# hkbharath/MARL-MASS

Hardware: AMD Instinct MI355X
Metric: agent-steps/sec (whole node), MASS CBF shield on, 65536 envs x 8 CAVs (higher is better)
Workload: dtype f64

## Files before the change

marl-mass_amd/csrc/mm_kernels.hip:

```cpp
#include <hip/hip_runtime.h>
#include <math.h>
#include <stdio.h>
#include <string.h>

#include <type_traits>

#include "mm_device.h"
#include "mm_div.h"
#include "mm_handle.h"
#define MM_COUNTS_FN __host__ __device__ inline
#include "../../include/mm_counts.h"
#include "../../include/mm_policy_wide.h"
#include "../../include/mm_env_params.h"

using namespace mm;

struct DevCfg {
  int env_kind, shield, nsub, T, action_masking, auto_reset, obs_f64, N, E, debug_flags, n_hdv;
  double dt, collision_reward, high_speed_reward, headway_cost, headway_time, merging_lane_cost;
  double rs_lo, rs_hi, eta, tau;
  double inv_dt, rs_span, rs_ispan, rs_span2, rs_ispan2;
  int agent_reward;
  int steer_vel;
  int *err;
// ... 1307 lines not shown
  } else {
    return c;
  }
}
template <int G, int SHIELD, bool MIXED>
#ifndef MM_GENERAL_NONE_WAVES
#define MM_GENERAL_NONE_WAVES 3
#endif
constexpr int step_min_waves(bool ipm = false) { return SHIELD == MM_SHIELD_NONE ? (G >= MM_NONE_WIDE_G ? 2 : (MIXED ? MM_GENERAL_NONE_WAVES : MM_NONE_WAVES)) : (ipm ? (G >= 6 ? MM_IPM_WIDE_WAVES : (MIXED ? MM_IPM_WAVES : MM_IPM_CAV_WAVES)) : MM_MIN_WAVES); }
template <int G, int KIND, int SHIELD, bool MIXED, bool IPM = false, bool TRACE = false, bool SPLIT = false, bool PENV = false>
#ifndef MM_STEP_BLOCK
#define MM_STEP_BLOCK 64
#endif
__global__ __launch_bounds__(MM_STEP_BLOCK, (SPLIT ? MM_SPLIT_WAVES : step_min_waves<G, SHIELD, MIXED>(IPM))) void step_kernel(DevCfg c, DevState st, const int32_t *__restrict__ actions,
                                                   MMStepOut out, double *metrics, SweepBuf sb, int kb, PoseBuf pb) {
  constexpr bool IDM = kIdm<KIND>;
  constexpr bool LC = (KIND == MM_ENV_V1) || IDM;
  constexpr bool SHIELDED = LC && (SHIELD != MM_SHIELD_NONE);
  static_assert(!IDM || (MIXED && SHIELD == MM_SHIELD_NONE && !IPM && !SPLIT), "hdv-v1: general unshielded kernels only");
  constexpr bool MASS = (SHIELD == MM_SHIELD_MASS);
  static_assert(!IPM || SHIELDED, "the IPM mode lives in shielded kernels");
  static_assert(!SPLIT || IPM, "the split form exists for the interior-point kernels");
  static_assert(!PENV || (SHIELDED && KIND == MM_ENV_V1 && !TRACE && !SPLIT), "per-env parameters: fused shielded v1 kernels without the trace");
#ifdef MM_SERIAL_ALL
  constexpr bool kSerialOnly = true || IPM;
#else
#ifdef MM_SERIAL_MASS
  constexpr bool kSerialOnly = MIXED || MASS || IPM;
#else
  constexpr bool kSerialOnly = MIXED;
#endif
#endif
  constexpr bool kSine = SHIELDED && !SPLIT && !MIXED && !IPM && !kSerialOnly && kPow2<G> && G <= 8;
  constexpr bool kScan = kScanSelects && !MIXED && !TRACE;
#ifndef MM_CARRY_POSE
#define MM_CARRY_POSE 1
#endif
  constexpr bool kCarry = kSine && MM_CARRY_POSE != 0;
#ifndef MM_PRIMARY_PRIOR
#define MM_PRIMARY_PRIOR 1
#endif
  constexpr bool kPrimary = kSine && !TRACE && kVetoPrior && MM_PRIMARY_PRIOR != 0;
#ifndef MM_SINE_CARRY
#define MM_SINE_CARRY 0
#endif
  constexpr bool kSineCarry = kPrimary && MM_SINE_CARRY != 0;
#ifndef MM_ACT_FRAME
#define MM_ACT_FRAME 1
#endif
  constexpr bool kActSel = kPrimary && MM_ACT_FRAME != 0;
  constexpr bool kEarly = kSine && MM_EARLY_LOADS != 0;
  constexpr bool kHBits = kSine && !TRACE && kPoseHBits;
  constexpr bool kWideObs = kSine && !TRACE && kObsWide;
  double car_sn = __builtin_nan("");
  (void)car_sn;
  static_assert(kPow2<G> || MM_STEP_BLOCK == 64, "rotation layouts: one wave per workgroup");
  const long long gtid = (long long)blockIdx.x * blockDim.x + threadIdx.x;
  constexpr int kTail = kPow2<G> ? 64 : (64 / G) * G;
  const bool tail = lane_id() >= kTail;
  const int gb = kPow2<G> ? (lane_id() & ~(G - 1)) : (tail ? kTail - G : lane_id() - lane_id() % G);
  const int a = kPow2<G> ? (int)(gtid % G) : lane_id() - gb;
  const long long e = kPow2<G> ? gtid / G : (tail ? (long long)st.E : (gtid >> 6) * (64 / G) + lane_id() / G);
  const bool valid = e < st.E && a < st.N;
  const long long i = e * st.N + a;
  const long long A = st.A;
  const double dt = c.dt;

#ifdef MM_STAMPS
  const unsigned long long _rec_t0 = __builtin_amdgcn_s_memtime(), _rec_rt0 = __builtin_amdgcn_s_memrealtime();
  unsigned long long _t_last = __builtin_amdgcn_s_memtime(), _t_acc = 0;
#endif
  Veh v;
  const bool sv = MIXED && KIND == MM_ENV_V1 && c.steer_vel != 0;
  int steps = 0, time = 0, n_merge = 0, episode = 0;
  int car_code = 0;
  long long car_kx = 0, car_ky = 0, car_kh = 0;
  double car_s = 0.0, car_c = 1.0;
  int act_raw = 1;
  (void)act_raw;
  if constexpr (kEarly) {
    if (valid) act_raw = actions[i];
    if (e < st.E) { n_merge = st.I[MM_E_N_MERGE * st.E + e]; episode = st.I[MM_E_EPISODE * st.E + e]; }
  }
  if constexpr (kCarry) {
    if (valid) {
      car_kx = __double_as_longlong(pb.F[PB_KX * A + i]); car_ky = __double_as_longlong(pb.F[PB_KY * A + i]);
      car_kh = __double_as_longlong(pb.F[PB_KH * A + i]);
      car_s = pb.F[PB_SIN * A + i]; car_c = pb.F[PB_COS * A + i]; car_code = pb.code[i];
    }
  }
  load_veh(st, i, valid, v, sv);
  if (e < st.E) {
    steps = st.I[MM_E_STEPS * st.E + e]; time = st.I[MM_E_TIME * st.E + e];
  }
  if (!MIXED && v.kind == 2) v.kind = 1;
  if (IDM && v.present) v.kind = 2;
  const bool hdv = MIXED && v.kind == 2;
  const bool ctrl = IDM ? v.present : (v.present && !hdv);
  const bool ctrl_x = IDM ? false : ctrl;
  int action;
  if constexpr (kEarly) action = ctrl ? act_raw : 1;
  else action = (!IDM && valid && ctrl) ? actions[i] : 1;
  if ((unsigned)action > 4u) {
    if (!SPLIT || kb == 0) atomicOr(c.err, MM_LATCH_BAD_ACTION);
    action = 1;
  }
  const unsigned present_bits = group_ballot<G>(v.present, gb);
  const unsigned ctrl_bits = group_ballot<G>(ctrl, gb);
  const int n_veh = __popc(present_bits), n_ctrl = __popc(ctrl_bits);
  if (!SPLIT || kb == 0) steps += 1;

  double cpsi = 1.0, spsi = 0.0;
  double st_t = __builtin_nan("");
  int pk_self = v.lane;
  bool carried = false;
  if constexpr (kCarry) {
    const bool hit = car_kx == __double_as_longlong(v.x) && car_ky == __double_as_longlong(v.y) && car_kh == __double_as_longlong(v.h) &&
                     (car_code >> 8) == ((kPoseWritten >> 8) | (MASS ? 1 : 0)) && (car_code & 7) == v.lane;
    carried = !__any(v.present && !hit);
    if (carried && v.present) { spsi = car_s; cpsi = car_c; pk_self = (car_code & 0xFF) | (kHBits ? pose_hbits(v.h) : 0); }
  }
  if (!carried) {
    if (v.present) mmm_sincos(v.h, &spsi, &cpsi);
    if (SHIELDED && v.present) pk_self = pose_code(v.lane, next_lane(v.lane, v.x, v.y), MASS ? corner_flags<kSine>(v.x, v.y, spsi, cpsi, v.lane) : 0);
    if constexpr (kHBits) { if (v.present) pk_self |= pose_hbits(v.h); }
  }

  enum { C_B = 0, C_H1X = 8, C_H1VX, C_H2X, C_H2VX, C_SSTEER, C_SACC, C_TSPEED, C_A = 15, C_GU0 = 23, C_GU1 = 24, C_PRE = 25, C_MSGW = 29 };
  constexpr bool kMailbox = G <= 8 || !kPow2<G>;
  constexpr bool kPackMsg = !kPow2<G>;
  constexpr int kColdB = kMailbox ? (kPackMsg ? 29 : 30) : 25;
  constexpr bool kRoomy = false;
  constexpr int C_CPSI = kColdB + G - 1, C_GVX = C_CPSI + 1;
  constexpr int kColdN = !SHIELDED ? 15 : (kSerialOnly ? 23 : kColdB + G - 1 + (kRoomy ? 2 : 0));
  static_assert(kColdN * MM_STEP_BLOCK * 8 >= (MM_STEP_BLOCK / 64) * 64 * 30 * 4, "the obs staging must fit in the cold slots");
  __shared__ alignas(kWideObs ? 16 : 8) double s_cold[kColdN][MM_STEP_BLOCK];
  const int tid = threadIdx.x;
  auto cold_i = [&](int slot, int col) -> int & { return ((int *)&s_cold[slot][col])[0]; };
  if (LC) {
    s_cold[C_H1X][tid] = v.h1x; s_cold[C_H1VX][tid] = v.h1vx; s_cold[C_H2X][tid] = v.h2x; s_cold[C_H2VX][tid] = v.h2vx;
    s_cold[C_SSTEER][tid] = v.safe_steer; s_cold[C_SACC][tid] = v.safe_acc;
  }
  s_cold[C_TSPEED][tid] = v.tspeed;
  if constexpr (kEarly) {
    static_assert(kMailbox && !kPackMsg, "the high words of the pose-code and rank-word slots must be free");
    ((int *)&s_cold[C_PRE + 3][tid])[1] = n_merge; ((int *)&s_cold[C_MSGW][tid])[1] = episode;
  }
  if constexpr (kRoomy) { s_cold[C_CPSI][tid] = cpsi; s_cold[C_GVX][tid] = v.gvx; }
  auto CPSI = [&]() -> double { if constexpr (kRoomy) return s_cold[C_CPSI][tid]; else return cpsi; };
  auto GVX = [&]() -> double { if constexpr (kRoomy) return s_cold[C_GVX][tid]; else return v.gvx; };
  bool env_active = IDM ? n_veh > 0 : n_ctrl > 0;
  if constexpr (SPLIT) {
    if (kb > 0) env_active = e < st.E && sb.envf[e] != 0;
  }
  STAMP(0);
  const int k_lo = SPLIT ? (kb > 0 ? kb - 1 : 0) : 0, k_hi = SPLIT ? (kb < c.nsub ? kb : c.nsub - 1) : c.nsub - 1;
  for (int k = k_lo; k <= k_hi; k++) {
    const bool head = !SPLIT || k == kb, tail = !SPLIT || k != kb;
    const bool live = env_active && v.present;
    QpTrace qt = {0, __builtin_nan(""), __builtin_nan(""), __builtin_nan(""), __builtin_nan(""),
                  __builtin_nan(""), __builtin_nan(""), __builtin_nan("")};
    int rank = 0;
    if ((SHIELDED || MIXED) && head) {
      for_partners<G>([&](auto mc) {
        constexpr int m = decltype(mc)::value;
        double px = px_d<m, G>(v.x, a);
        bool pp = px_i<m, G>((int)live, a) != 0;
        if constexpr (kScan) rank += (pp & ((px > v.x) | ((px == v.x) & (pidx<m, G>(a) < a)))) ? 1 : 0;
        else rank += (pp && (px > v.x || (px == v.x && pidx<m, G>(a) < a))) ? 1 : 0;
      });
    }
    if (head) v.tspeed = s_cold[C_TSPEED][tid];
    if constexpr (kActSel) {
      Veh w = v;
      if (time % c.nsub == 0) hl_act<KIND>(w, action);
      controlled_act<false, kSine>(w, -1, sv, st_t);
      v.hl = live ? w.hl : v.hl; v.sidx = live ? w.sidx : v.sidx; v.tspeed = live ? w.tspeed : v.tspeed;
      v.tlane = live ? w.tlane : v.tlane; v.act_acc = live ? w.act_acc : v.act_acc;
    } else {
      if (live && !hdv && head) {
        if (time % c.nsub == 0) hl_act<KIND>(v, action);
      }
    }
    const int tl_pre = v.tlane;
    if constexpr (!kActSel) {
      if (live && !hdv && head) controlled_act<!MIXED && !kPrimary, kSine>(v, -1, sv, st_t);
    }
    if (head) s_cold[C_TSPEED][tid] = v.tspeed;
    if constexpr (MIXED) { STAMP(1); }
    if constexpr (MIXED) {
      if (head && __any(hdv && live)) {
        const bool acting = hdv && live && !v.crashed;
        double koff = 0.0, koff_obst = 0.0;
        if (__any(acting && v.lane == MM_LANE_KB0)) {
          koff = kSineAmp * mmm_sin(kSinePuls * (v.x - lane_sx(MM_LANE_KB0)) + kSinePhase);
          koff_obst = kSineAmp * mmm_sin(kSinePuls * (kObstX - lane_sx(MM_LANE_KB0)) + kSinePhase);
        }
        Body self = {true, false, v.x, v.y, v.h, v.v, v.tspeed, v.lane, spsi, cpsi, koff};
        const double s_me = v.x - lane_sx(v.lane);
        NbSel n0 = {0, 0, -1, -1}, n1 = {0, 0, -1, -1};
        const LaneFrame lf0 = lane_frame(v.lane);
        if (acting && lane_after_end(v.tlane, v.x)) v.tlane = next_lane(v.tlane, v.x, v.y);
        const int my_tl = v.tlane;
        const bool lc_branch = v.lane != my_tl;
        const bool same_road = lane_road(v.lane) == lane_road(my_tl);
        const bool timer_due = !lc_branch && (1.0 < v.gvx);
        const int side = v.lane == MM_LANE_BC0 ? MM_LANE_BC1 : (v.lane == MM_LANE_BC1 ? MM_LANE_BC0 : -1);
        const bool try_mobil = acting && timer_due && side >= 0 && lane_reachable(side < 0 ? 0 : side, v.x, v.y);
        const int sl = side < 0 ? 0 : side;
        const double s_side = v.x - lane_sx(sl);
        const LaneFrame lf1 = lane_frame(sl);
        unsigned abort_mask = 0;
        for_partners<G>([&](auto mc) {
          constexpr int m = decltype(mc)::value;
          const int p = pidx<m, G>(a);
          const bool bp = px_i<m, G>((int)live, a) != 0;
          const double bx = px_d<m, G>(v.x, a), by = px_d<m, G>(v.y, a), bk = px_d<m, G>(koff, a);
          if (acting) {
            neighbour_update(lf0, s_me, bp, bx, by, bk, p, n0);
            if (try_mobil) neighbour_update(lf1, s_side, bp, bx, by, bk, p, n1);
          }
          if (__any(acting && lc_branch && same_road)) {
            Body b = {bp, false, bx, by, 0.0, px_d<m, G>(v.v, a), 0.0, px_i<m, G>(v.lane, a), px_d<m, G>(spsi, a), px_d<m, G>(cpsi, a), bk};
// ... 42 lines not shown
            const int p_tl = ((pk & 15) < rank) ? ((pk >> 8) & 7) : ((pk >> 4) & 7);
            hit = hit || (((abort_mask >> p) & 1u) && p_tl == my_tl);
          });
          const int nxt = (acting && lc_branch) ? ((same_road && hit) ? v.lane : my_tl) : tl_post;
          const bool changed = nxt != tl_post;
          tl_post = nxt;
          if (!__any(changed)) break;
        }
        if constexpr (MIXED) { STAMP(5); }
        if (acting) {
          v.tlane = tl_post;
          v.act_acc = clipd(acc_f0, -6.0, 6.0);
        }
      }
      if (head && live && (!hdv || !v.crashed)) steer_lane(v, sv && !hdv, st_t);
      if (head && hdv && live) v.gvx += dt;
    }
    bool first_B = false;
    if constexpr (kPrimary) {
      static_assert(!MIXED && !SPLIT, "kPrimary: no HDVs, no steer_vel, every launch a whole step");
      first_B = (c.debug_flags & 1) == 0 && live && v.hist_len >= 2 && (v.tlane != v.lane || v.crashed) && !(v.flags & MM_FLAG_IS_LC_SAFE);
      if (live) {
        const int tl_1 = v.tlane + (first_B ? v.lane - v.tlane : 0);
        const double steer = steering_control<kSine, kSineCarry>(v.x, v.y, v.h, v.v, tl_1, st_t, car_sn);
        v.act_steer = clipd(steer, -kPi / 3, kPi / 3);
        const double steer_1 = v.act_steer, st_t_1 = st_t;
        clip_actions<kSine>(v, LC, st_t);
        if (first_B) { v.act_steer = steer_1; st_t = st_t_1; }
      }
    } else {
      if (live && head) clip_actions<kSine>(v, LC && !hdv, st_t);
    }
    STAMP(1);
    Cand cA;
    memset(&cA, 0, sizeof cA);
    const bool shield_on = SHIELDED && live && !hdv && v.hist_len >= 2;
    if constexpr (kSineCarry) car_sn = __builtin_nan("");
    if (live && head) cA = predict<KIND, SHIELDED, MASS, MIXED, kSine, kHBits>(v, v.act_steer, st_t, spsi, cpsi, dt, sv && !hdv, kSineCarry ? &car_sn : nullptr);
    auto park = [&](auto base_c, const Cand &cc, double steer) {
      constexpr int base = decltype(base_c)::value;
      if constexpr (SHIELDED) {
        s_cold[base + 0][tid] = cc.x; s_cold[base + 1][tid] = cc.y; s_cold[base + 2][tid] = cc.h;
        cold_i(base + 3, tid) = cc.pk; s_cold[base + 4][tid] = cc.cpsi; s_cold[base + 5][tid] = steer;
        s_cold[base + 6][tid] = cc.gvx; s_cold[base + 7][tid] = cc.spsi;
      }
    };
    auto park_at = [&](int base, const Cand &cc, double steer) {
      s_cold[base + 0][tid] = cc.x; s_cold[base + 1][tid] = cc.y; s_cold[base + 2][tid] = cc.h;
      cold_i(base + 3, tid) = cc.pk; s_cold[base + 4][tid] = cc.cpsi; s_cold[base + 5][tid] = steer;
      s_cold[base + 6][tid] = cc.gvx; s_cold[base + 7][tid] = cc.spsi;
    };
    if constexpr (kPrimary) park_at(first_B ? (int)C_B : (int)C_A, cA, v.act_steer);
    else if (head) park(std::integral_constant<int, C_A>{}, cA, v.act_steer);
    STAMP(2);
    const bool needB = SHIELDED && shield_on && (v.tlane != v.lane || v.crashed || sv);
    bool haveB = first_B, haveA = !first_B;
    (void)haveA;
    auto make_other = [&]() {
      if constexpr (kPrimary) {
        const bool mk_A = !haveA;
        if (mk_A || (needB && !haveB)) {
          double t_o;
          const int tl_o = v.lane + (mk_A ? v.tlane - v.lane : 0);
          double steer_o = steering_control<kSine>(v.x, v.y, v.h, v.v, tl_o, t_o);
          if (mk_A) {
            steer_o = clipd(steer_o, -kPi / 3, kPi / 3);
            if (v.crashed) { steer_o = 0; t_o = 0; }
          }
          park_at(mk_A ? (int)C_A : (int)C_B, predict<KIND, true, MASS, MIXED, kSine, kHBits>(v, steer_o, t_o, spsi, cpsi, dt, false), steer_o);
          haveA = true; haveB = haveB || !mk_A;
        }
      }
    };
    auto make_B = [&]() {
      if constexpr (SHIELDED) {
        if (needB && !haveB) {
          double tB;
          double steerB = steering_control<kSine>(v.x, v.y, v.h, v.v, v.lane, tB);
          if (sv) steerB = steer_vel_command(steerB, v.sang);
          park(std::integral_constant<int, C_B>{}, predict<KIND, true, MASS, MIXED, kSine, kHBits>(v, steerB, tB, spsi, CPSI(), dt, sv), steerB);
          haveB = true;
        }
      }
    };
    auto chosen = [&](bool useB) {
      if constexpr (!SHIELDED) {
        return cA;
      } else {
        const int base = useB ? C_B : C_A;
        Cand cc;
        cc.x = s_cold[base + 0][tid]; cc.y = s_cold[base + 1][tid]; cc.h = s_cold[base + 2][tid];
        cc.gvx = s_cold[base + 6][tid]; cc.cpsi = s_cold[base + 4][tid]; cc.spsi = s_cold[base + 7][tid];
        const int pk = cold_i(base + 3, tid);
        cc.pk = pk; cc.lane = pk & 7;
        return cc;
      }
    };
    if constexpr (SPLIT) {
      if (!head && live && valid) {
        v.act_acc = sw_f(sb, SW_ACCN, a, e);
        if (MIXED && hdv) {
          v.act_steer = sw_f(sb, SW_ASTEER, a, e);
          if (sw_i(sb, SW_RES, a, e) & 16) s_cold[C_H1X][tid] = sw_f(sb, SW_ACC, a, e);
        }
        s_cold[C_A + 0][tid] = sw_f(sb, SW_AX, a, e); s_cold[C_A + 1][tid] = sw_f(sb, SW_AY, a, e); s_cold[C_A + 2][tid] = sw_f(sb, SW_AH, a, e);
        cold_i(C_A + 3, tid) = sw_i(sb, SW_APK, a, e); s_cold[C_A + 4][tid] = sw_f(sb, SW_ACPSI, a, e); s_cold[C_A + 5][tid] = sw_f(sb, SW_ASTEER, a, e);
// ... 14 lines not shown
#endif
    if constexpr (kPrimary) {
      use_B = first_B;
#ifdef MM_STAMPS
      st_prior = first_B;
#endif
      CAND_COUNT(MM_CS_FIRST_B, first_B);
    } else if constexpr (SHIELDED && !SPLIT && !kSerialOnly && kVetoPrior) {
      CAND_COUNT(MM_CS_UPFRONT, (c.debug_flags & 1) == 0 && shield_on && needB && !(v.flags & MM_FLAG_IS_LC_SAFE));
      if ((c.debug_flags & 1) == 0 && shield_on && needB && !(v.flags & MM_FLAG_IS_LC_SAFE)) { make_B(); use_B = true; }
#ifdef MM_STAMPS
      st_prior = use_B;
#endif
    }
    STAMP(MM_CS_UPFRONT_CYCLES);
    if constexpr (SPLIT) {
      if (head) {
        make_B();
        if constexpr (!kSerialOnly && kVetoPrior) use_B = (c.debug_flags & 1) == 0 && shield_on && needB && !(v.flags & MM_FLAG_IS_LC_SAFE);
        const int n_live = __popc(group_ballot<G>(live, gb));
        if (valid) {
          sw_i(sb, SW_META, a, e) = (live ? 1 : 0) | (shield_on ? 2 : 0) | (needB ? 4 : 0) | (hdv ? 8 : 0) | (use_B ? 16 : 0) | (v.flags & 255) << 8 | (v.hl & 255) << 16;
          if (live) {
            sw_i(sb, SW_WPK, a, e) = pk_self;
            sw_f(sb, SW_CPSI, a, e) = cpsi; sw_f(sb, SW_ACCN, a, e) = v.act_acc;
            sw_f(sb, SW_AX, a, e) = cA.x; sw_f(sb, SW_AY, a, e) = cA.y; sw_f(sb, SW_AH, a, e) = cA.h; sw_i(sb, SW_APK, a, e) = cA.pk;
            sw_f(sb, SW_ACPSI, a, e) = cA.cpsi; sw_f(sb, SW_AGVX, a, e) = cA.gvx; sw_f(sb, SW_ASTEER, a, e) = v.act_steer; sw_f(sb, SW_ASPSI, a, e) = cA.spsi;
            if (needB) {
              sw_f(sb, SW_BX, a, e) = s_cold[C_B + 0][tid]; sw_f(sb, SW_BY, a, e) = s_cold[C_B + 1][tid]; sw_f(sb, SW_BH, a, e) = s_cold[C_B + 2][tid];
              sw_i(sb, SW_BPK, a, e) = cold_i(C_B + 3, tid); sw_f(sb, SW_BCPSI, a, e) = s_cold[C_B + 4][tid]; sw_f(sb, SW_BSTEER, a, e) = s_cold[C_B + 5][tid];
              sw_f(sb, SW_BGVX, a, e) = s_cold[C_B + 6][tid]; sw_f(sb, SW_BSPSI, a, e) = s_cold[C_B + 7][tid];
            }
            sb.order[(long long)rank * sb.Ep + e] = (uint8_t)a;
          }
          if (a >= n_live) sb.order[(long long)a * sb.Ep + e] = 0xFF;
          if (a == 0) sb.envf[e] = env_active ? 1 : 0;
        }
      } else if (shield_on && valid) {
        const int res = sw_i(sb, SW_RES, a, e);
        new_acc = sw_f(sb, SW_ACC, a, e); veto = (res & 2) != 0; use_B = (res & 4) != 0; new_flags = (res >> 8) & 255;
      }
    }

    if constexpr (SHIELDED) {
     if (__any(shield_on) && (!SPLIT || head)) {
      bool serial = !SPLIT && (kSerialOnly || (c.debug_flags & 1) != 0);
      ShieldOut so;
      memset(&so, 0, sizeof so);
      if constexpr (!kSerialOnly) {
       if (!serial) {
        static_assert(!MIXED || kSerialOnly, "the parallel form is CAV-only (the twin branch needs the literal sweep)");
        bool irregular = false;
        constexpr bool count5 = G > 4;
        if constexpr (kMailbox) { s_cold[C_PRE + 0][tid] = v.x; s_cold[C_PRE + 1][tid] = v.y; s_cold[C_PRE + 2][tid] = v.h; cold_i(C_PRE + 3, tid) = pk_self; }
        double qc_h0 = 0.0, qc_h3 = 0.0, qc_d = 0.0;
        int qc_meta = 0;
        (void)qc_h0; (void)qc_h3; (void)qc_d; (void)qc_meta;
        for (int pass = 0; pass <= st.N; pass++) {
#ifdef MM_STAMPS
#ifdef MM_COUNT_ROUNDS
          if ((threadIdx.x & 63) == 13) _t_acc += (pass == 0 ? 1ull << 32 : 0ull);
#else
          if ((threadIdx.x & 63) == 13) _t_acc += 1 + (pass == 0 ? 1ull << 32 : 0ull);
#endif
#endif
          const double mine_gvx = s_cold[(use_B ? C_B : C_A) + 6][tid];
          const double h1vx_mine = s_cold[C_H1VX][tid];
          s_cold[C_GU0][tid] = slot_gu<MASS>(s_cold[C_H2VX][tid], MASS ? s_cold[C_SACC][tid] : kCbfAccLo, GVX(), dt);
          s_cold[C_GU1][tid] = slot_gu<MASS>(h1vx_mine, kCbfAccLo, mine_gvx, dt);
          if constexpr (kMailbox) {
            const int my_word = (live ? rank : 99) | (use_B ? 256 : 0);
            if constexpr (kPackMsg) ((int *)&s_cold[C_PRE + 3][tid])[1] = my_word;
            else cold_i(C_MSGW, tid) = my_word;
            __builtin_amdgcn_fence(__ATOMIC_RELEASE, "wavefront");
            __builtin_amdgcn_wave_barrier();
            __builtin_amdgcn_fence(__ATOMIC_ACQUIRE, "wavefront");
          }
          Cand mine;
          if constexpr (!kMailbox) mine = chosen(use_B);
          double k_ol = INFINITY, k_oa = INFINITY, k_oar = INFINITY;
          int j_ol = -1, j_oa = -1, j_oar = -1;
          for_partners<G>([&](auto mc) {
            constexpr int m = decltype(mc)::value;
            const int p = pidx<m, G>(a);
            int p_rank, opk;
            double ox, oy, oh;
            bool i_first;
            if constexpr (kMailbox) {
              const int pl = plane<m, G>(tid, a);
              int pw;
              if constexpr (kPackMsg) pw = ((const int *)&s_cold[C_PRE + 3][pl])[1];
              else pw = cold_i(C_MSGW, pl);
              p_rank = pw & 255;
              i_first = live && rank < p_rank;
              const int pb = (!i_first && p_rank < 99) ? ((pw & 256) ? (int)C_B : (int)C_A) : (int)C_PRE;
              ox = s_cold[pb + 0][pl]; oy = s_cold[pb + 1][pl];
              if constexpr (kHBits) oh = 0.0;
              else oh = s_cold[pb + 2][pl];
              opk = cold_i(pb + 3, pl) | (p_rank < 99 ? 256 : 0);
            } else {
              p_rank = dppx_i<m>(live ? rank : 99);
              i_first = live && rank < p_rank;
              const double sx_ = i_first ? mine.x : v.x, sy_ = i_first ? mine.y : v.y, sh_ = i_first ? mine.h : v.h;
              const int spk = i_first ? mine.pk : pk_self;
              ox = dppx_d<m>(sx_); oy = dppx_d<m>(sy_); oh = dppx_d<m>(sh_);
              opk = dppx_i<m>(spk | (int)live << 8);
            }
            const bool o_first = !i_first && p_rank < 99;
            const Rel r = relate<kHBits && kMailbox>(v.x, v.y, pk_self, ((opk >> 8) & 1) != 0, ox, oy, oh, opk);
            if constexpr (count5) s_cold[kColdB + m - 1][tid] = r.key;
            const bool b_ol = (r.cls == 1) & ((r.key < k_ol) | ((r.key == k_ol) & (p < (j_ol & 15))));
            const bool b_oa = (r.cls == 2) & ((r.key < k_oa) | ((r.key == k_oa) & (p < (j_oa & 15))));
            const bool b_oar = (r.cls == 3) & ((r.key < k_oar) | ((r.key == k_oar) & (p < (j_oar & 15))));
            const int pf = p | (o_first ? 16 : 0) | (r.cflag ? 32 : 0);
            k_ol = b_ol ? r.key : k_ol; j_ol = b_ol ? pf : j_ol;
            k_oa = b_oa ? r.key : k_oa; j_oa = b_oa ? pf : j_oa;
            k_oar = b_oar ? r.key : k_oar; j_oar = b_oar ? pf : j_oar;
          });
          const bool ol_first = j_ol >= 0 && (j_ol & 16), oa_first = j_oa >= 0 && (j_oa & 16), oar_stepped = j_oar >= 0 && (j_oar & 16);
          const bool cadj = j_oa >= 0 && (j_oa & 32);
          j_ol = j_ol < 0 ? -1 : (j_ol & 15); j_oa = j_oa < 0 ? -1 : (j_oa & 15); j_oar = j_oar < 0 ? -1 : (j_oar & 15);
          STAMP(3);
          Neigh nb;
          memset(&nb, 0, sizeof nb);
          nb.has_ol = j_ol >= 0; nb.has_oa = j_oa >= 0; nb.has_oar = j_oar >= 0;
          if constexpr (count5) {
            int pos_ol = 0, pos_oa = 0, pos_oar = 0;
#pragma unroll
            for (int m = 1; m < G; m++) {
              const int p = pidx_rt<G>(a, m);
              const double km = s_cold[kColdB + m - 1][tid];
              pos_ol += (km < k_ol || (km == k_ol && p < j_ol)) ? 1 : 0;
              pos_oa += (km < k_oa || (km == k_oa && p < j_oa)) ? 1 : 0;
              pos_oar += (km < k_oar || (km == k_oar && p < j_oar)) ? 1 : 0;
            }
            nb.has_ol = nb.has_ol && pos_ol < 5;
            nb.has_oa = nb.has_oa && pos_oa < 5;
            nb.has_oar = nb.has_oar && pos_oar < 5;
          }
          nb.constrain_adj = MASS && nb.has_oa && cadj;
          if constexpr (SPLIT) {
            if (valid && shield_on)
              sw_i(sb, SW_CLS, a, e) = (j_ol & 15) | (j_oa & 15) << 4 | (j_oar & 15) << 8 | (nb.has_ol ? 1 << 12 : 0) | (nb.has_oa ? 1 << 13 : 0) |
                                       (nb.has_oar ? 1 << 14 : 0) | (nb.constrain_adj ? 1 << 15 : 0);
            break;
          }
          __builtin_amdgcn_fence(__ATOMIC_RELEASE, "wavefront");
          __builtin_amdgcn_wave_barrier();
          __builtin_amdgcn_fence(__ATOMIC_ACQUIRE, "wavefront");
          const int t_ol = tid - a + (j_ol < 0 ? a : j_ol), t_oa = tid - a + (j_oa < 0 ? a : j_oa);
          nb.ol_x = s_cold[ol_first ? C_H1X : C_H2X][t_ol]; nb.ol_gu = s_cold[ol_first ? C_GU1 : C_GU0][t_ol];
          nb.oa_x = s_cold[oa_first ? C_H1X : C_H2X][t_oa]; nb.oa_gu = s_cold[oa_first ? C_GU1 : C_GU0][t_oa];
          const int src_ol = gb + (j_ol < 0 ? 0 : j_ol), src_oa = gb + (j_oa < 0 ? 0 : j_oa), src_oar = gb + (j_oar < 0 ? 0 : j_oar);
          const double cpsi_now = CPSI();
          nb.oar_x = shfl_d(v.x, src_oar); nb.oar_vx = shfl_d(v.v * cpsi_now, src_oar);
          bool ol_dyn = MASS && nb.has_ol && ol_first, oa_dyn = MASS && nb.has_oa && oa_first;
          {
            unsigned rep = obstacle_override<MASS>(nb, v.x, v.y);
            if (rep & 1u) ol_dyn = false;
            if (rep & 2u) oa_dyn = false;
          }
          irregular = irregular || (shield_on && nb.has_oar && oar_stepped);
// ... 83 lines not shown
#endif
            for (int round = 0; round <= st.N; round++) {
#if defined(MM_STAMPS) && defined(MM_COUNT_ROUNDS)
              if ((threadIdx.x & 63) == 13) _t_acc += 1;
#endif
              CAND_COUNT(MM_CS_ROUNDS, shield_on);
              const double gu_cur = slot_gu<true>(h1vx_mine, acc_cur, mine_gvx, dt);
              const double da = shfl_d(gu_cur, src_ol), db = shfl_d(gu_cur, src_oa);
              if (ol_dyn) nb.ol_gu = da;
              if (oa_dyn) nb.oa_gu = db;
              rr = shield_rows<true>(c, ss, nb);
              d_cur = qp_exact(ss, rr);
              double acc_next = v.act_acc;
              if (shield_on) {
                if (slow_lc) acc_next = shield_post<true>(env_cfg<PENV>(c, e, st.E), v, ss, rr, d_cur, true, false).acc;
                else acc_next = div_c((ss.u0 + d_cur) - ss.evx, dt, c.inv_dt);
              }
              const bool changed = __double_as_longlong(acc_next) != __double_as_longlong(acc_cur);
              acc_cur = acc_next;
              if (!__any(changed)) break;
            }
            so = shield_post<true>(env_cfg<PENV>(c, e, st.E), v, ss, rr, d_cur, true, false);
            STAMP(MM_CS_ROUND_CYCLES);
          } else {
          for (int round = 0; round <= st.N; round++) {
            if (MASS) {
              const double gu_cur = slot_gu<true>(h1vx_mine, acc_cur, mine_gvx, dt);
              const double da = shfl_d(gu_cur, src_ol), db = shfl_d(gu_cur, src_oa);
              if (ol_dyn) nb.ol_gu = da;
              if (oa_dyn) nb.oa_gu = db;
            }
            so = shield_dyn<MASS, true, false>(env_cfg<PENV>(c, e, st.E), v, ss, nb, shield_on);
            const double acc_next = shield_on ? so.acc : v.act_acc;
            const bool changed = __double_as_longlong(acc_next) != __double_as_longlong(acc_cur);
            acc_cur = acc_next;
            if (!MASS || !__any(changed)) break;
          }
          }
          }
          if (TRACE && shield_on) trace_status(out.trace + (long long)k * MM_T_COUNT * A + i, A, so);
          STAMP(4);
          const bool want_B = shield_on && so.veto && needB;
          CAND_COUNT(MM_CS_LAZY_B, want_B && !haveB);
          if constexpr (kPrimary) {
            CAND_COUNT(MM_CS_LAZY_A, !want_B && !haveA);
            if (want_B ? !haveB : !haveA) make_other();
          } else {
            if (want_B) make_B();
          }
          STAMP(5);
          const bool flip = want_B != use_B;
          use_B = want_B;
          if (!__any(flip)) break;
        }
        serial = __any(irregular);
        if (!serial && shield_on) {
          new_acc = so.acc; veto = so.veto; new_flags = so.flags; qt = so.qt;
          if (IPM && so.bounds) atomicOr(c.err, MM_LATCH_QP_BOUNDS);
        }
       }
      }
      if (!SPLIT && serial) {
        CAND_COUNT(MM_CS_FALLBACK, !haveA || (needB && !haveB));
        if constexpr (kPrimary) make_other();
        else make_B();
        use_B = false; veto = false; new_acc = v.act_acc; new_flags = v.flags;
        if constexpr (kRoomy) { v.gvx = GVX(); cpsi = CPSI(); }
        double wx = v.x, wy = v.y, wh = v.h, wg = hdv ? 1.0 : v.gvx, wacc = hdv ? kCbfAccLo : s_cold[C_SACC][tid], wvx = v.v * cpsi;
        double whx = s_cold[C_H2X][tid], whvx = s_cold[C_H2VX][tid];
        int wpk = pk_self;
        if (MIXED && hdv && live) {
        }
        double wgu = slot_gu<MASS>(whvx, MASS ? wacc : kCbfAccLo, wg, dt);
        bool w_stepped = false;
        double twin_shift = 0;
        int srank = 0;
        for_partners<G>([&](auto mc) {
          constexpr int m = decltype(mc)::value;
          srank += (px_i<m, G>(shield_on ? rank : 99, a) < rank) ? 1 : 0;
        });
        for (int j = 0; j < st.N; j++) {
          const unsigned sel = group_ballot<G>(shield_on && srank == j, gb);
          if (!__any(sel != 0)) break;
          const bool has = sel != 0;
          const int ai = has ? (__ffs((int)sel) - 1) : 0;
          const int src = gb + ai;
          if constexpr (MIXED) {
            const int r_ego = shfl_i(rank, src);
            if (live && hdv && has && rank < r_ego && !w_stepped) {
              const Cand ca = chosen(false);
              wx = ca.x; wy = ca.y; wh = ca.h; wpk = ca.pk;
              whx = s_cold[C_H1X][tid]; whvx = s_cold[C_H1VX][tid]; w_stepped = true; twin_shift = 0;
              wgu = slot_gu<MASS>(whvx, MASS ? wacc : kCbfAccLo, wg, dt);
            }
          }
          const double ex = shfl_d(v.x, src), ey = shfl_d(v.y, src);
          const int epk = shfl_i(pk_self, src);
          const double e_vx = shfl_d(v.v * cpsi, src);
          const Rel rl = relate(ex, ey, epk, live && has && a != ai, wx, wy, wh, wpk, hdv);
          int pos = 0;
          for_partners<G>([&](auto mc) {
            constexpr int m = decltype(mc)::value;
            double kp = px_d<m, G>(rl.key, a);
            pos += (kp < rl.key || (kp == rl.key && pidx<m, G>(a) < a)) ? 1 : 0;
          });
          const bool in5 = rl.key < INFINITY && pos < 5;
// ... 72 lines not shown
    CAND_COUNT(MM_CS_PRIOR_HELD, st_prior && use_B);
    CAND_COUNT(MM_CS_PRIOR_LIFTED, st_prior && !use_B);
    if (SPLIT && SHIELDED && out.trace && live && tail && !shield_on) {
      out.trace[(long long)k * MM_T_COUNT * A + i + MM_T_QP_ROWS * A] = 0;
    }
    if (!SPLIT && SHIELDED && TRACE && live) {
      double *t = out.trace + (long long)k * MM_T_COUNT * A + i;
      t[MM_T_QP_ROWS * A] = qt.rows; t[MM_T_QP_A * A] = qt.a;
      t[MM_T_QP_H0 * A] = qt.h0; t[MM_T_QP_H1 * A] = qt.h1; t[MM_T_QP_H2 * A] = qt.h2;
      t[MM_T_QP_H3 * A] = qt.h3; t[MM_T_QP_D * A] = qt.d; t[MM_T_LC_MARGIN * A] = qt.margin;
    }
    if (tail) {
    if constexpr (kSineCarry) {
      if (!(live && use_B == first_B)) car_sn = __builtin_nan("");
    }
    if (live) {
      const Cand cc = chosen(use_B);
      const double acc = (SHIELDED && shield_on) ? new_acc : v.act_acc;
      double nv = v.v + acc * dt;
      nv = nv > 0 ? nv : 0;
      if (SHIELDED && shield_on) {
        if (veto) v.tlane = v.lane;
        v.flags = new_flags;
      }
      v.x = cc.x; v.y = cc.y; v.h = cc.h; v.v = nv; v.lane = cc.lane;
      if (LC) {
        if (!hdv) {
          double steer_nom = v.act_steer;
          if constexpr (SHIELDED) steer_nom = s_cold[C_A + 5][tid];
          s_cold[C_SSTEER][tid] = (SHIELDED && shield_on && veto && haveB) ? s_cold[C_B + 5][tid] : steer_nom;
          s_cold[C_SACC][tid] = acc; v.gvx = cc.gvx;
          if constexpr (kRoomy) s_cold[C_GVX][tid] = cc.gvx;
          if (sv) v.sang += s_cold[C_SSTEER][tid] * dt;
        }
        s_cold[C_H2X][tid] = s_cold[C_H1X][tid]; s_cold[C_H2VX][tid] = s_cold[C_H1VX][tid];
        s_cold[C_H1X][tid] = v.x; s_cold[C_H1VX][tid] = v.v * cc.cpsi;
        if (v.hist_len < 2) v.hist_len++;
      }
      if constexpr (kRoomy) s_cold[C_CPSI][tid] = cc.cpsi;
      else cpsi = cc.cpsi;
      spsi = cc.spsi;
      if (SHIELDED) pk_self = cc.pk;
    }

    STAMP(7);
    unsigned need = 0;
#ifdef MM_STAMPS
    bool near_any = false;
    CAND_COUNT(MM_CS_PRECHECK, live);
#endif
    for_partners<G>([&](auto mc) {
      constexpr int m = decltype(mc)::value;
      double px = px_d<m, G>(v.x, a), py = px_d<m, G>(v.y, a), ph = px_d<m, G>(v.h, a);
      bool pp = px_i<m, G>((int)live, a) != 0;
      double dx = px - v.x, dy = py - v.y;
      const bool near = live & pp & !((dx * dx + dy * dy) > kU5);
      CAND_COUNT(MM_CS_NEAR, near);
#ifdef MM_STAMPS
      near_any |= near;
#endif
      need |= (near & boxes_may_touch(dx, dy, v.h, ph, 0.9 * kVehLength / 2, 0.9 * kVehWidth / 2)) ? 1u << pidx<m, G>(a) : 0u;
    });
    CAND_COUNT(MM_CS_NEAR_ANY, near_any);
    {
      double dx = kObstX - v.x, dy = kObstY - v.y;
      const bool near = live & !((dx * dx + dy * dy) > kU5);
      need |= (near & boxes_may_touch(dx, dy, v.h, 0.0, 0.9 * 2.0 / 2, 0.9 * 2.0 / 2)) ? 1u << G : 0u;
    }
    unsigned hits = 0;
    bool obst_hit = false;
    if (__any(need != 0)) {
      for (int p = 0; p <= G; p++) {
        const bool t = ((need >> p) & 1u) != 0;
        if (!__any(t)) continue;
        const bool is_obst = p == G;
        const int src = gb + (is_obst ? 0 : p);
        double px = shfl_d(v.x, src), py = shfl_d(v.y, src), ph = shfl_d(v.h, src);
        if (is_obst) { px = kObstX; py = kObstY; ph = 0.0; }
        const double ol = is_obst ? 2.0 : kVehLength, ow = is_obst ? 2.0 : kVehWidth;
        if (t && rects_intersect(v.x, v.y, v.h, px, py, ol, ow, ph)) {
          if (is_obst) obst_hit = true;
          else hits |= 1u << p;
        }
      }
    }
    if (__any(hits != 0 || obst_hit)) {
      unsigned cb = group_ballot<G>(v.crashed != 0, gb);
      const unsigned ob = group_ballot<G>(obst_hit, gb);
      for (int ii = 0; ii < st.N; ii++) {
        const unsigned row = (unsigned)shfl_i((int)hits, gb + ii);
        for (int jj = 0; jj < st.N; jj++) {
          const double si = shfl_d(v.v, gb + ii), sj = shfl_d(v.v, gb + jj);
          const bool fire = !((cb >> ii) & 1u) && ii != jj && ((row >> jj) & 1u);
          if (fire) {
            const double s = fabs(si) <= fabs(sj) ? si : sj;
            if (a == ii || a == jj) { v.v = s; v.crashed = 1; }
            cb |= (1u << ii) | (1u << jj);
          }
        }
        if (!((cb >> ii) & 1u) && ((ob >> ii) & 1u)) {
          if (a == ii) { v.v = fabs(v.v) <= 0 ? v.v : 0.0; v.crashed = 1; }
          cb |= 1u << ii;
        }
      }
    }
    STAMP(8);
    if (env_active) time += 1;
// ... 88 lines not shown
  double local = 0;
  if (ctrl) {
    const bool xrew = LC && c.agent_reward != 0, is_mrew = c.agent_reward == 2;
    const bool half = xrew && is_mrew && (v.flags & MM_FLAG_IS_COLLABORATING);
    double scaled = 0 + (half ? div_c((v.v - c.rs_lo) * (1 - 0), c.rs_span2, c.rs_ispan2)
                              : div_c((v.v - c.rs_lo) * (1 - 0), c.rs_span, c.rs_ispan));
    double merging = 0;
    if (v.lane == MM_LANE_BC1 && (!(xrew && is_mrew) || (v.flags & MM_FLAG_IS_LC_SAFE))) {
      double t = v.x - 420;
      merging = -mmm_exp(MM_DIVC(-(t * t), 1000.0));
    }
    double hc = v.v > 0 ? mmm_log(hd / (env_cfg<PENV>(c, e, st.E).headway_time * v.v)) : 0;
    if (xrew) hc = -1 * hc;
    local = c.collision_reward * (-1 * v.crashed) + (c.high_speed_reward * clipd(scaled, 0, 1)) +
            c.merging_lane_cost * merging + c.headway_cost * (hc < 0 ? hc : 0);
  }
  double regional = 0;
  {
    const bool on_main = v.lane == MM_LANE_AB0 || v.lane == MM_LANE_BC0 || v.lane == MM_LANE_CD0;
    const int i_fl = on_main ? of_i : sf_i, i_rl = on_main ? or_i : sr_i;
    const int i_fr = on_main ? sf_i : of_i, i_rr = on_main ? sr_i : or_i;
    const double r_fl = shfl_d(local, gb + (i_fl < 0 ? 0 : i_fl)), r_fr = shfl_d(local, gb + (i_fr < 0 ? 0 : i_fr));
    const double r_rl = shfl_d(local, gb + (i_rl < 0 ? 0 : i_rl)), r_rr = shfl_d(local, gb + (i_rr < 0 ? 0 : i_rr));
    auto is_mdp = [&](int j) { return j >= 0 && !((hdv_bits >> j) & 1u); };
    double sum = 0;
    int cnt = 0;
    if (is_mdp(i_fl)) { sum += r_fl; cnt++; }
    if (is_mdp(i_fr)) { sum += r_fr; cnt++; }
    sum += local; cnt++;
    if (is_mdp(i_rl)) { sum += r_rl; cnt++; }
    if (is_mdp(i_rr)) { sum += r_rr; cnt++; }
    regional = sum / cnt;
  }
  double rsum = 0, ssum = 0, tsum = 0;
#pragma unroll
  for (int q = 0; q < G; q++) {
    const double lr = shfl_d(local, gb + q), sp = shfl_d(v.v, gb + q);
    const bool in = q < st.N, cq = in & (((ctrl_bits >> q) & 1u) != 0), pq = in & (((present_bits >> q) & 1u) != 0);
    const double r1 = rsum + lr, s1 = ssum + sp, t1 = tsum + sp;
    rsum = cq ? r1 : rsum; ssum = cq ? s1 : ssum;
    tsum = pq ? t1 : tsum;
  }
  const double reward = env_ok ? rsum / n_ctrl : 0, avg_speed = env_ok ? ssum / n_ctrl : 0;
  const double traffic_speed = env_ok ? tsum / n_veh : 0;
  double th = INFINITY;
  if (ctrl) {
    double h2d = hd;
    if (fabs(kObstY - v.y) <= 2 && kObstX > v.x) { double dd = kObstX - v.x; if (dd < h2d) h2d = dd; }
    h2d = h2d - kVehLength;
    double vx = v.v * cpsi;
    th = h2d / (vx > 1 ? vx : 1);
  }
  const double min_headway = group_min_d<G>(th, a);
  if constexpr (kEarly) { n_merge = ((const int *)&s_cold[C_PRE + 3][tid])[1]; episode = ((const int *)&s_cold[C_MSGW][tid])[1]; }
  else if (e < st.E) { n_merge = st.I[MM_E_N_MERGE * st.E + e]; episode = st.I[MM_E_EPISODE * st.E + e]; }
  double merge_pct = __builtin_nan("");
  if (done) {
    const int n_rem = __popc(group_ballot<G>(
        ctrl && (v.lane == MM_LANE_BC1 || v.lane == MM_LANE_KB0 || v.lane == MM_LANE_JK0), gb));
    merge_pct = n_merge > 0 ? (double)(n_merge - n_rem) / n_merge * 100 : 100.0;
  }
  if (valid) {
    if (out.agents_rewards) out.agents_rewards[i] = ctrl ? local : 0;
    if (out.regional_rewards) out.regional_rewards[i] = ctrl ? regional : 0;
    if (out.agents_dones) out.agents_dones[i] = ctrl ? (uint8_t)(v.crashed || steps >= c.T || v.x < 0) : 1;
    if (out.crashed) out.crashed[i] = v.present ? (uint8_t)v.crashed : 0;
    if (out.agents_info) {
      out.agents_info[i * 3 + 0] = v.present ? v.x : 0;
      out.agents_info[i * 3 + 1] = v.present ? v.y : 0;
      out.agents_info[i * 3 + 2] = v.present ? v.v : 0;
    }
  }
  if (e < st.E && a == 0 && env_ok) {
    if (out.reward) out.reward[e] = reward;
    if (out.done) out.done[e] = (uint8_t)done;
    if (out.average_speed) out.average_speed[e] = avg_speed;
    if (out.traffic_speed) out.traffic_speed[e] = traffic_speed;
    if (out.min_headway) out.min_headway[e] = min_headway;
    if (out.merge_percent) out.merge_percent[e] = merge_pct;
  }
  STAMP(10);
  if (metrics) {
    static_assert(MM_STEP_BLOCK % 64 == 0, "whole waves per workgroup");
    const bool lead = e < st.E && a == 0 && env_ok;
    const double mv[8] = {lead ? reward : 0.0, (lead && done && crashed_bits) ? 1.0 : 0.0, lead ? avg_speed : 0.0,
                          lead ? traffic_speed : 0.0, lead ? 1.0 : 0.0, (lead && done) ? merge_pct : 0.0,
                          (lead && done) ? 1.0 : 0.0, lead ? min_headway : INFINITY};
    if (a == 0) {
#pragma unroll
      for (int k = 0; k < 8; k++) s_cold[C_B + k][tid] = mv[k];
    }
    __builtin_amdgcn_fence(__ATOMIC_RELEASE, "wavefront");
    __builtin_amdgcn_wave_barrier();
    __builtin_amdgcn_fence(__ATOMIC_ACQUIRE, "wavefront");
    const int ln = lane_id();
    if (ln < 8) {
      const int slot = C_B + ln, base = tid - ln;
      double acc = ln == 7 ? INFINITY : 0.0;
#pragma unroll
      for (int j = 0; j < 64 / G; j++) {
        const double x = s_cold[slot][base + j * G];
        acc = ln == 7 ? fmin(acc, x) : acc + x;
      }
      double *row = metrics + (gtid >> 6) * 8;
      if ((c.debug_flags >> kMetricsAccBit) & 1) {
        if (ln == 7) (void)unsafeAtomicMin(&row[7], acc);
        else (void)unsafeAtomicAdd(&row[ln], acc);
// ... 1355 lines not shown
```

Baseline: 2.634 billion.

## Encode partner rank order and liveness as per-lane bitmask, drop mailbox rank word

The first partner sweep now builds a bitmask of which partners rank ahead and which are live, instead of only counting rank. The mailbox layout is reorganized so each lane reads the partner's pre-step or post-step pose directly by bit selection, which removes the rank/use_B message word and the heading load. The saved liveness bits also replace a cross-lane exchange in the collision pre-check. The cost is extra LDS slots, plus rewriting the post pose whenever use_B flips.

New measurement: 2.704 billion, median of 6. 1.03x the previous value.

```diff
diff --git a/marl-mass_amd/csrc/mm_kernels.hip b/marl-mass_amd/csrc/mm_kernels.hip
--- a/marl-mass_amd/csrc/mm_kernels.hip
+++ b/marl-mass_amd/csrc/mm_kernels.hip
@@ -1383,6 +1383,14 @@
   constexpr bool kEarly = kSine && MM_EARLY_LOADS != 0;
   constexpr bool kHBits = kSine && !TRACE && kPoseHBits;
   constexpr bool kWideObs = kSine && !TRACE && kObsWide;
+#ifndef MM_PARTNER_BITS
+#define MM_PARTNER_BITS 1
+#endif
+  constexpr bool kPBits = kPrimary && kHBits && kEarly && !PENV && MM_PARTNER_BITS != 0;
+#ifndef MM_PARTNER_LIVE
+#define MM_PARTNER_LIVE 1
+#endif
+  constexpr bool kPLive = kPBits && MM_PARTNER_LIVE != 0;
   double car_sn = __builtin_nan("");
   (void)car_sn;
   static_assert(kPow2<G> || MM_STEP_BLOCK == 64, "rotation layouts: one wave per workgroup");
@@ -1457,10 +1465,11 @@
     if constexpr (kHBits) { if (v.present) pk_self |= pose_hbits(v.h); }
   }
 
-  enum { C_B = 0, C_H1X = 8, C_H1VX, C_H2X, C_H2VX, C_SSTEER, C_SACC, C_TSPEED, C_A = 15, C_GU0 = 23, C_GU1 = 24, C_PRE = 25, C_MSGW = 29 };
+  enum { C_B = 0, C_H1X = 8, C_H1VX, C_H2X, C_H2VX, C_SSTEER, C_SACC, C_TSPEED, C_A = 15, C_GU0 = 23, C_GU1 = kPBits ? 27 : 24,
+         C_PRE = kPBits ? 24 : 25, C_PREPK = C_PRE + (kPBits ? 2 : 3), C_POST = C_PRE + 4, C_MSGW = 29 };
   constexpr bool kMailbox = G <= 8 || !kPow2<G>;
   constexpr bool kPackMsg = !kPow2<G>;
-  constexpr int kColdB = kMailbox ? (kPackMsg ? 29 : 30) : 25;
+  constexpr int kColdB = kPBits ? 31 : (kMailbox ? (kPackMsg ? 29 : 30) : 25);
   constexpr bool kRoomy = false;
   constexpr int C_CPSI = kColdB + G - 1, C_GVX = C_CPSI + 1;
   constexpr int kColdN = !SHIELDED ? 15 : (kSerialOnly ? 23 : kColdB + G - 1 + (kRoomy ? 2 : 0));
@@ -1475,7 +1484,7 @@
   s_cold[C_TSPEED][tid] = v.tspeed;
   if constexpr (kEarly) {
     static_assert(kMailbox && !kPackMsg, "the high words of the pose-code and rank-word slots must be free");
-    ((int *)&s_cold[C_PRE + 3][tid])[1] = n_merge; ((int *)&s_cold[C_MSGW][tid])[1] = episode;
+    ((int *)&s_cold[C_PREPK][tid])[1] = n_merge; ((int *)&s_cold[kPBits ? C_POST + 2 : C_MSGW][tid])[1] = episode;
   }
   if constexpr (kRoomy) { s_cold[C_CPSI][tid] = cpsi; s_cold[C_GVX][tid] = v.gvx; }
   auto CPSI = [&]() -> double { if constexpr (kRoomy) return s_cold[C_CPSI][tid]; else return cpsi; };
@@ -1492,14 +1501,21 @@
     QpTrace qt = {0, __builtin_nan(""), __builtin_nan(""), __builtin_nan(""), __builtin_nan(""),
                   __builtin_nan(""), __builtin_nan(""), __builtin_nan("")};
     int rank = 0;
+    int pbits = 0;
+    (void)pbits;
     if ((SHIELDED || MIXED) && head) {
       for_partners<G>([&](auto mc) {
         constexpr int m = decltype(mc)::value;
         double px = px_d<m, G>(v.x, a);
         bool pp = px_i<m, G>((int)live, a) != 0;
-        if constexpr (kScan) rank += (pp & ((px > v.x) | ((px == v.x) & (pidx<m, G>(a) < a)))) ? 1 : 0;
+        if constexpr (kPBits) pbits |= ((pp & ((px > v.x) | ((px == v.x) & (pidx<m, G>(a) < a)))) ? 1 << m : 0) | (pp ? 256 << m : 0);
+        else if constexpr (kScan) rank += (pp & ((px > v.x) | ((px == v.x) & (pidx<m, G>(a) < a)))) ? 1 : 0;
         else rank += (pp && (px > v.x || (px == v.x && pidx<m, G>(a) < a))) ? 1 : 0;
       });
+    }
+    if constexpr (kPBits) {
+      rank = __popc(pbits & 255);
+      pbits = live ? pbits : ((pbits >> 8) * 257);
     }
     if (head) v.tspeed = s_cold[C_TSPEED][tid];
     if constexpr (kActSel) {
@@ -1648,6 +1664,7 @@
     };
     if constexpr (kPrimary) park_at(first_B ? (int)C_B : (int)C_A, cA, v.act_steer);
     else if (head) park(std::integral_constant<int, C_A>{}, cA, v.act_steer);
+    if constexpr (kPBits) { s_cold[C_POST + 0][tid] = cA.x; s_cold[C_POST + 1][tid] = cA.y; cold_i(C_POST + 2, tid) = cA.pk; }
     STAMP(2);
     const bool needB = SHIELDED && shield_on && (v.tlane != v.lane || v.crashed || sv);
     bool haveB = first_B, haveA = !first_B;
@@ -1768,7 +1785,8 @@
         static_assert(!MIXED || kSerialOnly, "the parallel form is CAV-only (the twin branch needs the literal sweep)");
         bool irregular = false;
         constexpr bool count5 = G > 4;
-        if constexpr (kMailbox) { s_cold[C_PRE + 0][tid] = v.x; s_cold[C_PRE + 1][tid] = v.y; s_cold[C_PRE + 2][tid] = v.h; cold_i(C_PRE + 3, tid) = pk_self; }
+        if constexpr (kPBits) { s_cold[C_PRE + 0][tid] = v.x; s_cold[C_PRE + 1][tid] = v.y; cold_i(C_PREPK, tid) = pk_self; }
+        else if constexpr (kMailbox) { s_cold[C_PRE + 0][tid] = v.x; s_cold[C_PRE + 1][tid] = v.y; s_cold[C_PRE + 2][tid] = v.h; cold_i(C_PRE + 3, tid) = pk_self; }
         double qc_h0 = 0.0, qc_h3 = 0.0, qc_d = 0.0;
         int qc_meta = 0;
         (void)qc_h0; (void)qc_h3; (void)qc_d; (void)qc_meta;
@@ -1785,9 +1803,11 @@
           s_cold[C_GU0][tid] = slot_gu<MASS>(s_cold[C_H2VX][tid], MASS ? s_cold[C_SACC][tid] : kCbfAccLo, GVX(), dt);
           s_cold[C_GU1][tid] = slot_gu<MASS>(h1vx_mine, kCbfAccLo, mine_gvx, dt);
           if constexpr (kMailbox) {
-            const int my_word = (live ? rank : 99) | (use_B ? 256 : 0);
-            if constexpr (kPackMsg) ((int *)&s_cold[C_PRE + 3][tid])[1] = my_word;
-            else cold_i(C_MSGW, tid) = my_word;
+            if constexpr (!kPBits) {
+              const int my_word = (live ? rank : 99) | (use_B ? 256 : 0);
+              if constexpr (kPackMsg) ((int *)&s_cold[C_PRE + 3][tid])[1] = my_word;
+              else cold_i(C_MSGW, tid) = my_word;
+            }
             __builtin_amdgcn_fence(__ATOMIC_RELEASE, "wavefront");
             __builtin_amdgcn_wave_barrier();
             __builtin_amdgcn_fence(__ATOMIC_ACQUIRE, "wavefront");
@@ -1802,6 +1822,15 @@
             int p_rank, opk;
             double ox, oy, oh;
             bool i_first;
+            (void)p_rank; (void)i_first;
+            bool o_first, other;
+            if constexpr (kPBits) {
+              const int pl = plane<m, G>(tid, a);
+              const int pb = C_PRE + ((pbits >> m) & 1) * 4;
+              ox = s_cold[pb + 0][pl]; oy = s_cold[pb + 1][pl]; oh = 0.0;
+              opk = cold_i(pb + 2, pl);
+              o_first = ((pbits >> m) & 1) != 0; other = ((pbits >> (8 + m)) & 1) != 0;
+            } else {
             if constexpr (kMailbox) {
               const int pl = plane<m, G>(tid, a);
               int pw;
@@ -1822,8 +1851,10 @@
               ox = dppx_d<m>(sx_); oy = dppx_d<m>(sy_); oh = dppx_d<m>(sh_);
               opk = dppx_i<m>(spk | (int)live << 8);
             }
-            const bool o_first = !i_first && p_rank < 99;
-            const Rel r = relate<kHBits && kMailbox>(v.x, v.y, pk_self, ((opk >> 8) & 1) != 0, ox, oy, oh, opk);
+            o_first = !i_first && p_rank < 99;
+            other = ((opk >> 8) & 1) != 0;
+            }
+            const Rel r = relate<kHBits && kMailbox>(v.x, v.y, pk_self, other, ox, oy, oh, opk);
             if constexpr (count5) s_cold[kColdB + m - 1][tid] = r.key;
             const bool b_ol = (r.cls == 1) & ((r.key < k_ol) | ((r.key == k_ol) & (p < (j_ol & 15))));
             const bool b_oa = (r.cls == 2) & ((r.key < k_oa) | ((r.key == k_oa) & (p < (j_oa & 15))));
@@ -2013,6 +2044,13 @@
           const bool flip = want_B != use_B;
           use_B = want_B;
           if (!__any(flip)) break;
+          if constexpr (kPBits) {
+            if (flip) {
+              const int cb = use_B ? (int)C_B : (int)C_A;
+              s_cold[C_POST + 0][tid] = s_cold[cb + 0][tid]; s_cold[C_POST + 1][tid] = s_cold[cb + 1][tid];
+              cold_i(C_POST + 2, tid) = cold_i(cb + 3, tid);
+            }
+          }
         }
         serial = __any(irregular);
         if (!serial && shield_on) {
@@ -2191,7 +2229,9 @@
     for_partners<G>([&](auto mc) {
       constexpr int m = decltype(mc)::value;
       double px = px_d<m, G>(v.x, a), py = px_d<m, G>(v.y, a), ph = px_d<m, G>(v.h, a);
-      bool pp = px_i<m, G>((int)live, a) != 0;
+      bool pp;
+      if constexpr (kPLive) pp = ((pbits >> (8 + m)) & 1) != 0;
+      else pp = px_i<m, G>((int)live, a) != 0;
       double dx = px - v.x, dy = py - v.y;
       const bool near = live & pp & !((dx * dx + dy * dy) > kU5);
       CAND_COUNT(MM_CS_NEAR, near);
@@ -2386,7 +2426,7 @@
     th = h2d / (vx > 1 ? vx : 1);
   }
   const double min_headway = group_min_d<G>(th, a);
-  if constexpr (kEarly) { n_merge = ((const int *)&s_cold[C_PRE + 3][tid])[1]; episode = ((const int *)&s_cold[C_MSGW][tid])[1]; }
+  if constexpr (kEarly) { n_merge = ((const int *)&s_cold[C_PREPK][tid])[1]; episode = ((const int *)&s_cold[kPBits ? C_POST + 2 : C_MSGW][tid])[1]; }
   else if (e < st.E) { n_merge = st.I[MM_E_N_MERGE * st.E + e]; episode = st.I[MM_E_EPISODE * st.E + e]; }
   double merge_pct = __builtin_nan("");
   if (done) {
```
